# jyakaranda/A-LeGO-LOAM

Hardware: AMD Instinct MI355X
Metric: scans/sec (16x1800 LiDAR) full IP->LO->LM loop (higher is better)
Workload: dtype f32/f64

## Files before the change

a-lego-loam_amd/csrc/alego_api.hip:

```cpp
#include <hip/hip_runtime.h>

#include <cmath>
#include <cstdio>
#include <cstdlib>
#include <algorithm>
#include <cstring>
#include <mutex>
#include <string>
#include <vector>

#include "../../include/alego_mi355x.h"
#include "dev_common.h"
#include "guard_alloc.h"
#include "lm_host.h"
#include "prof.h"
#include "voxel.h"

thread_local Profiler* g_prof = nullptr;


void launch_ip(const DevCtx& d, int ring_pos, bool want_labels, hipStream_t st);
void launch_fe(const DevCtx& d, hipStream_t st);
void launch_lo(const DevCtx& d, hipStream_t st);
void launch_lo_grid(const DevCtx& d, hipStream_t st);
// ... 1166 lines not shown
  hipSetDevice(h->device);
  return lm_host_map_get_keyframe(h->lm, slot, id, out, &h->err);
}
int alego_map_assemble(alego_handle* h, int slot, int kinds, float leaf, alego_point* out, int32_t cap) {
  if (int r = check_slot(h, slot)) return r;
  hipSetDevice(h->device);
  g_prof = &h->prof;
  return lm_host_map_assemble(h->lm, slot, kinds, leaf, out, cap, &h->err);
}
int alego_map_get_stamps(alego_handle* h, int slot, int32_t first, int32_t n, double* out) {
  if (int r = check_slot(h, slot)) return r;
  hipSetDevice(h->device);
  return lm_host_map_stamps(h->lm, slot, first, n, out, 0, &h->err);
}
int alego_map_set_stamps(alego_handle* h, int slot, int32_t first, int32_t n, const double* stamps) {
  if (int r = check_slot(h, slot)) return r;
  hipSetDevice(h->device);
  return lm_host_map_stamps(h->lm, slot, first, n, const_cast<double*>(stamps), 1, &h->err);
}
int alego_map_keyposes(alego_handle* h, int slot, alego_point* out, int32_t cap) {
  if (int r = check_slot(h, slot)) return r;
  hipSetDevice(h->device);
  return lm_host_map_keyposes(h->lm, slot, out, cap, &h->err);
}
int alego_lm_get_local_map(alego_handle* h, int slot, alego_point* corner, int32_t corner_cap, alego_point* surf, int32_t surf_cap, int32_t n_out[2]) {
  if (int r = check_slot(h, slot)) return r;
  if (!n_out || corner_cap < 0 || surf_cap < 0) return ALEGO_ERR_ARG;
  hipSetDevice(h->device);
  return lm_host_get_local_map(h->lm, slot, corner, corner_cap, surf, surf_cap, n_out, &h->err);
}
int alego_voxel_grid(alego_handle* h, const alego_point* pts, int32_t n, float leaf, alego_point* out, int32_t cap) {
  if (!h || n < 0 || cap < 0 || (n > 0 && !pts) || !(leaf > 0.f)) return ALEGO_ERR_ARG;
  hipSetDevice(h->device);
  g_prof = &h->prof;
  return lm_host_voxel_grid(h->lm, h->stream, pts, n, leaf, out, cap, &h->err);
}

int alego_debug_get(alego_handle* h, int slot, const char* name, void* out, int cap_bytes, int* count, int* dtype) {
  if (int r = check_slot(h, slot)) return r;
  hipSetDevice(h->device);
  const DevCtx& d = h->d;
  int sc[SC_COUNT];
  HIP_TRY(h, hipMemcpyAsync(sc, d.scal + (size_t)slot * SC_COUNT, sizeof(sc), hipMemcpyDeviceToHost, stream_of(h, slot)));
  HIP_TRY(h, hipStreamSynchronize(stream_of(h, slot)));
  const std::string s(name);
  const size_t base = (size_t)slot * d.N;
  const int M = sc[SC_M];
  const int cur = sc[SC_CUR];
  int fc[8];
  HIP_TRY(h, hipMemcpy(fc, d.feat_cnt + (size_t)slot * 8, sizeof(fc), hipMemcpyDeviceToHost));
  const void* src = nullptr;
  size_t n = 0;
  int dt = 0, esz = 4;
  auto set = [&](const void* p, size_t cnt, int t) { src = p; n = cnt; dt = t; esz = t == 1 ? 8 : t == 3 ? 1 : 4; };
  if (s == "range_img") set(d.range_img + base, d.N, 0);
  else if (s == "label_img") set(d.label_img + base, d.N, 2);
  else if (s == "flag_img") set(d.flag_img + base, d.N, 3);
  else if (s == "owner") set(d.owner + base, d.N, 2);
  else if (s == "parent") set(d.parent + base, d.N, 2);
  else if (s == "seg_cloud") set(d.seg_pts + base, (size_t)M * 4, 0);
  else if (s == "outlier") set(d.outlier + base, (size_t)sc[SC_NOUT] * 4, 0);
  else if (s == "undistorted" && d.P.deskew_mode) set(d.seg_dsk + base, (size_t)sc[SC_M_DSK] * 4, 0);
  else if (s == "imu_ptr") set(d.imu_ptr + (size_t)slot * 4, 3, 2);
  else if (s == "imu_ring") set(d.imu_ring + (size_t)slot * ALEGO_IMU_Q * 10, ALEGO_IMU_Q * 10, 1);
  else if (s == "seg_ground") set(d.seg_ground + base, M, 3);
  else if (s == "seg_col") set(d.seg_col + base, M, 2);
  else if (s == "seg_range") set(d.seg_range + base, M, 0);
  else if (s == "ring_start") set(d.ring_start + (size_t)slot * d.NS, d.NS, 2);
  else if (s == "ring_end") set(d.ring_end + (size_t)slot * d.NS, d.NS, 2);
  else if (s == "orientation") set(d.ori + (size_t)slot * 4, 3, 0);
  else if (s == "scal") set(d.scal + (size_t)slot * SC_COUNT, SC_COUNT, 2);
  else if (s == "curv_d") set(d.cd + base, M, 0);
  else if (s == "picked_occl") set(d.picked0 + base, M, 3);
  else if (s == "point_label") set(d.plabel + base, M, 2);
  else if (s == "sharp") set(d.feat[0] + ((size_t)slot * 2 + cur) * d.fcap[0], (size_t)fc[cur * 4 + 0] * 4, 0);
  else if (s == "less_sharp") set(d.feat[1] + ((size_t)slot * 2 + cur) * d.fcap[1], (size_t)fc[cur * 4 + 1] * 4, 0);
  else if (s == "flat") set(d.feat[2] + ((size_t)slot * 2 + cur) * d.fcap[2], (size_t)fc[cur * 4 + 2] * 4, 0);
  else if (s == "less_flat") set(d.feat[3] + ((size_t)slot * 2 + cur) * d.fcap[3], (size_t)fc[cur * 4 + 3] * 4, 0);
  else if (s == "sharp_idx") set(d.feat_idx[0] + ((size_t)slot * 2 + cur) * d.fcap[0], fc[cur * 4 + 0], 2);
  else if (s == "less_sharp_idx") set(d.feat_idx[1] + ((size_t)slot * 2 + cur) * d.fcap[1], fc[cur * 4 + 1], 2);
  else if (s == "flat_idx") set(d.feat_idx[2] + ((size_t)slot * 2 + cur) * d.fcap[2], fc[cur * 4 + 2], 2);
  else if (s == "lo_surf_corr") set(d.lo_corr + (size_t)slot * (d.lo_qcap_surf + d.lo_qcap_corner) * 4, (size_t)fc[cur * 4 + 2] * 4, 2);
  else if (s == "lo_corner_corr") set(d.lo_corr + ((size_t)slot * (d.lo_qcap_surf + d.lo_qcap_corner) + d.lo_qcap_surf) * 4, (size_t)fc[cur * 4 + 0] * 4, 2);
  else if (s == "lo_state") set(d.lo_state + (size_t)slot * LO_STATE_N, LO_STATE_N, 1);
  else if (s == "poses") set(d.poses + (size_t)slot * 16, 16, 1);
  else return lm_host_debug_get(h->lm, slot, name, out, cap_bytes, count, dtype, &h->err);
  if ((size_t)cap_bytes < n * esz) { h->err = "debug_get: buffer too small"; return ALEGO_ERR_CAPACITY; }
  if (n) HIP_TRY(h, hipMemcpy(out, src, n * esz, hipMemcpyDeviceToHost));
  *count = (int)n; *dtype = dt;
  return 0;
}

}
```

a-lego-loam_amd/csrc/kernels_fe2.hip:

```cpp
#include <algorithm>
#include <cstdlib>
#include "dev_common.h"
#include "prof.h"
#include "vgrid.h"

#define FE_MAXH 4096

#ifndef FF_G
#define FF_G 4
#endif
#define FF_LPR (64 / FF_G)
#define FF_HALO 8
#define FF_Q0 64
#ifndef FC_NW
#define FC_NW 4
#endif

struct FfLayout {
  int scap, mch, wave_bytes;
};
__host__ __device__ inline FfLayout ff_layout(int sector_cap) {
  FfLayout L;
  L.scap = (FF_Q0 + sector_cap + FF_HALO + 63) & ~63;
  L.mch = L.scap / 64 + 1;
// ... 213 lines not shown
    uint32_t bk = 0u, bp = 0u;
    for (int t = gl; t < nwave; t += FF_LPR) {
      if (act && t < ncand) {
        const uint2 e = lp[t * dir];
        const bool take = FLAT ? e.x > bk : e.x >= bk;
        bk = take ? e.x : bk; bp = take ? e.y : bp;
      }
    }
    const uint32_t kmax = group_max_u32<64 / FF_G>(bk);
    act = act && kmax != 0u;
    if (!__any(act)) break;
    uint32_t pm = group_max_u32<64 / FF_G>(bk == kmax ? bp : 0u);
    if (FLAT) pm = ~pm;
    const int c = (int)(pm >> 6), rf = (int)((pm >> 3) & 7u), rb = (int)(pm & 7u);
    picked += act ? 1 : 0;
    int lab;
    bool spread, more;
    ff_label<FLAT>(P, picked, nmax, lab, spread, more);
    const int lo = max(c - (spread ? rb : 0), 0), hi = c + (spread ? rf : 0);
    const bool rem = act && (FLAT || lab != 0);
    for (int t = gl; t < nwave; t += FF_LPR) {
      if (rem && t < ncand) {
        const uint32_t pv = lp[t * dir].y, loc = (FLAT ? ~pv : pv) >> 6;
        if (loc - (uint32_t)lo <= (uint32_t)(hi - lo)) lp[t * dir].x = 0u;
      }
    }
    ff_commit<FLAT>(R, rem, lab, c, lo, hi, mark, mw, gl);
    act = act && more;
  }
}

#define FF_MW_MAX 28
template <bool BIG>
__global__ void __launch_bounds__(64) fe_pickc(DevCtx d, int sector_cap) {
  const int slot = blockIdx.y + d.slot0, ring0 = blockIdx.x * FF_G, lane = threadIdx.x;
  const int g = lane / FF_LPR, gl = lane % FF_LPR;
  const int NS = d.NS;
  const alego_params& P = d.P;
  int* sc = d.scal + slot * SC_COUNT;
  __shared__ uint32_t s_mark[FF_G][FF_MW_MAX];
  const int mw = min((sector_cap + FF_HALO + 31) / 32 + 1, FF_MW_MAX);
  if (blockIdx.x == 0 && lane == 0) { sc[SC_FE_EPOCH] = sc[SC_FE_EPOCH] + 1; sc[SC_FE_TICKET] = 0; }
  const int ring = ring0 + g;
  const bool rv = ring < NS;
  const int rc = rv ? ring : 0;
  const int S = rv ? d.ring_start[slot * NS + ring] : 0, E = rv ? d.ring_end[slot * NS + ring] : 0;
  int* st = d.st_idx + ((size_t)slot * NS + rc) * d.st_stride;
  const int* cc = ff_counts(d, slot, rc);
  FfPick R;
  R.act0 = false; R.sp = 0; R.carry = -1; R.carry_in = -1; R.n_sharp = 0; R.n_ls = 0; R.n_flat = 0;
  R.st_sharp = st; R.st_lsharp = st + d.cap_sharp; R.st_flat = st + d.cap_sharp + d.cap_lsharp;
  uint32_t* mk = s_mark[g];
  const int NSEC = P.n_sectors;
  for (int j = 0; j < NSEC; ++j) {
    int sp = 0, ep = -1;
    if (rv) ff_sector(P, S, E, j, sp, ep);
    R.act0 = rv && sp < ep; R.sp = sp; R.carry_in = R.carry;
    const int ns = R.act0 ? cc[2 * j] : 0, nf = R.act0 ? cc[2 * j + 1] : 0;
    uint2* lst = ff_list(d, slot, rc, j, sector_cap);
    for (int w = gl; w < mw; w += FF_LPR) mk[w] = 0u;
    const int nsw = (int)wave_max_u32((uint32_t)ns), nfw = (int)wave_max_u32((uint32_t)nf);
    constexpr int KU = 32 / FF_LPR;
    if (nsw <= (BIG ? 64 : 32)) ff_pick_regs<(BIG ? 2 : 1) * KU, false>(P, R, ns, lst, 1, mk, mw, gl);
    else if (nsw <= (BIG ? 128 : 64)) ff_pick_regs<(BIG ? 4 : 2) * KU, false>(P, R, ns, lst, 1, mk, mw, gl);
    else if (nsw <= (BIG ? 192 : 96) && !d.opt_fe_cand) ff_pick_regs<(BIG ? 6 : 3) * KU, false>(P, R, ns, lst, 1, mk, mw, gl);
    else ff_pick_mem<false>(P, R, ns, nsw, lst, 1, mk, mw, gl);
    __builtin_amdgcn_wave_barrier();
    if (nfw <= 32 && !(d.opt_fe_cand && nfw > 8)) ff_pick_regs<KU, true>(P, R, nf, lst + sector_cap - 1, -1, mk, mw, gl);
    else if (BIG && nfw <= 64 && !d.opt_fe_cand) ff_pick_regs<2 * KU, true>(P, R, nf, lst + sector_cap - 1, -1, mk, mw, gl);
    else ff_pick_mem<true>(P, R, nf, nfw, lst + sector_cap - 1, -1, mk, mw, gl);
    __builtin_amdgcn_wave_barrier();
  }
  if (rv && gl == 0) {
    int* c = d.st_cnt + ((size_t)slot * NS + ring) * 8;
    c[0] = R.n_sharp; c[1] = R.n_ls; c[2] = R.n_flat;
  }
}

#ifndef FO_BLOCK
#define FO_BLOCK 256
#endif
#define FO_NB 256
#define FO_U 4
#define FO_CAP_PCT 72
#define FO_INVALID 0xFFFFFFFFu
#define FO_END 0xFFFFu
#define FO_SPIN_LIMIT (1 << 22)
#define FO_ALIAS_INTS (6 * ((FE_MAXH + LO_CH - 1) / LO_CH) > 768 ? 6 * ((FE_MAXH + LO_CH - 1) / LO_CH) : 768)
#define FO_STATIC_LDS (928 + 4 * FO_ALIAS_INTS)
#ifndef FO_BUDGET_BIG
#define FO_BUDGET_BIG 53248
#endif
#ifndef FO_KEYED
#define FO_KEYED 1
#endif
#ifndef FO_STAGE
#define FO_STAGE 0
#endif
struct FoLayout { int cap; int keyed; };
__host__ __device__ inline FoLayout fo_layout(int H) {
  const int budget = 12 * H + FO_STATIC_LDS > 40960 ? FO_BUDGET_BIG : 40960;
  FoLayout L;
  L.keyed = FO_KEYED && 14 * H + FO_STATIC_LDS <= budget;
  const int by_pct = (H * FO_CAP_PCT / 100 + 15) & ~15, by_lds = (budget - FO_STATIC_LDS - (L.keyed ? 14 : 12) * H) / 16;
  L.cap = !FO_STAGE || by_lds <= 0 ? 0 : (by_pct < by_lds ? by_pct : (by_lds & ~15));
  return L;
}
static size_t fo_lds_bytes(int H) { const FoLayout L = fo_layout(H); return std::max((size_t)(L.keyed ? 14 : 12) * H + (size_t)16 * L.cap, (size_t)6 * 65 * 4); }

DEV_INLINE uint32_t mad_u24(uint32_t a, uint32_t b, uint32_t c) { uint32_t r; asm("v_mad_u32_u24 %0, %1, %2, %3" : "=v"(r) : "v"(a), "v"(b), "v"(c)); return r; }

DEV_INLINE uint32_t fo_ord(float f) { const uint32_t b = (uint32_t)d_f2i(f); return b ^ ((b >> 31) ? 0xFFFFFFFFu : 0x80000000u); }
DEV_INLINE float fo_unord(uint32_t u) { return d_i2f((int32_t)(u ^ ((u >> 31) ? 0x80000000u : 0xFFFFFFFFu))); }

#ifdef ALEGO_TIMING
__device__ long long fo_times[24];
extern "C" void alego_fo_times(long long* out) { (void)hipMemcpyFromSymbol(out, HIP_SYMBOL(fo_times), sizeof(long long) * 24); }
#ifndef FO_TICK_RING
#define FO_TICK_RING 8
#endif
#define FO_TICK(k) do { if (threadIdx.x == 0 && ring == FO_TICK_RING && blockIdx.x == 0) fo_times[k] = wall_clock64(); } while (0)
#elif defined(FO_STOP_AFTER)
#define FO_TICK(k) do { if ((k) == FO_STOP_AFTER) { if (threadIdx.x == 0) __hip_atomic_store(&d.fe_sync[(size_t)slot * NS + ring], (epoch << 16), __ATOMIC_RELAXED, __HIP_MEMORY_SCOPE_AGENT); return; } } while (0)
#else
#define FO_TICK(k)
#endif

DEV_INLINE void fo_picks_out(const DevCtx& d, int slot, unsigned char* smem) {
  const int tid = threadIdx.x, NS = d.NS;
  const size_t base = (size_t)slot * d.N;
  const size_t fb = (size_t)slot * 2 + cur_in_flight(d, slot);
  const int* allc = d.st_cnt + (size_t)slot * NS * 8;
  const float4* seg = d.seg_lo + base;
  int (*s_off)[65] = reinterpret_cast<int (*)[65]>(smem);
  if (tid < 64) {
    const int r = tid;
    int c[4];
    c[0] = r < NS ? allc[r * 8 + 0] : 0; c[1] = r < NS ? allc[r * 8 + 1] : 0; c[2] = r < NS ? allc[r * 8 + 2] : 0;
    c[3] = (c[1] + LO_CH - 1) / LO_CH;
#pragma unroll
    for (int k = 0; k < 4; ++k) {
      const int incl = wave_incl_scan(c[k]);
      s_off[k][r] = incl - c[k];
      if (r == 63) s_off[k][64] = incl;
    }
  }
  __syncthreads();
  if (tid <= NS) {
    d.ring_off[(fb * 2) * (NS + 1) + tid] = tid < NS ? s_off[1][tid] : s_off[1][64];
    d.ring_boff[(fb * 2) * (NS + 1) + tid] = tid < NS ? s_off[3][tid] : s_off[3][64];
  }
  if (tid < 3) d.feat_cnt[fb * 4 + tid] = s_off[tid][64];
  auto ring_of = [&](int k, int i) -> int {
    int lo = 0, hi = NS - 1;
    while (lo < hi) { const int mid = (lo + hi + 1) >> 1; if (s_off[k][mid] <= i) lo = mid; else hi = mid - 1; }
    return lo;
  };
  const int stoff[3] = {0, d.cap_sharp, d.cap_sharp + d.cap_lsharp};
#pragma unroll
  for (int k = 0; k < 3; ++k) {
    float4* dst = d.feat[k] + fb * d.fcap[k];
    int* dsti = d.feat_idx[k] + fb * d.fcap[k];
    float4* bx = d.lo_box + (fb * 2 + 1) * d.lo_box_cap * 2;
    const bool boxes = k == F_LSHARP;
    const int nwork = boxes ? s_off[3][64] * LO_CH : s_off[k][64];
    for (int i0 = 0; i0 < nwork; i0 += FO_BLOCK) {
      int i = i0 + tid, r = 0, j = 0, bxi = 0;
      bool v = i < nwork;
      if (boxes) {
        bxi = min(i / LO_CH, s_off[3][64] - 1);
        r = ring_of(3, bxi); j = (bxi - s_off[3][r]) * LO_CH + (tid % LO_CH);
        v = v && j < s_off[k][r + 1] - s_off[k][r];
        i = s_off[k][r] + j;
      } else if (v) { r = ring_of(k, i); j = i - s_off[k][r]; }
      float4 p = make_float4(0.f, 0.f, 0.f, 0.f);
      if (v) {
        const int idx = d.st_idx[((size_t)slot * NS + r) * d.st_stride + stoff[k] + j];
        p = seg[idx];
        dsti[i] = idx; dst[i] = p;
      }
      if (boxes) {
        float mn[3] = {3.402823466e+38f, 3.402823466e+38f, 3.402823466e+38f}, mx[3] = {-3.402823466e+38f, -3.402823466e+38f, -3.402823466e+38f};
        if (v) { mn[0] = mx[0] = p.x; mn[1] = mx[1] = p.y; mn[2] = mx[2] = p.z; }
#pragma unroll
        for (int a = 0; a < 3; ++a)
          bfly_minmax_f32<LO_CH>(mn[a], mx[a]);
        if ((tid % LO_CH) == 0 && v) {
          bx[2 * bxi] = make_float4(mn[0], mn[1], mn[2], __int_as_float(i));
          bx[2 * bxi + 1] = make_float4(mx[0], mx[1], mx[2], __int_as_float(min(LO_CH, s_off[k][r + 1] - i)));
        }
      }
    }
  }
  if (d.n_launch == 1) {
    const int M = d.scal[slot * SC_COUNT + SC_M];
    for (int k = tid; k < M; k += FO_BLOCK) d.plabel[base + k] = 0;
    __syncthreads();
    for (int pass = 0; pass < 3; ++pass) {
      const int k = pass == 0 ? 1 : (pass == 1 ? 0 : 2), lab = pass == 0 ? 1 : (pass == 1 ? 2 : -1);
      for (int i = tid; i < s_off[k][64]; i += FO_BLOCK) {
        const int r = ring_of(k, i);
        d.plabel[base + d.st_idx[((size_t)slot * NS + r) * d.st_stride + stoff[k] + i - s_off[k][r]]] = lab;
      }
      __syncthreads();
    }
  }
}

__global__ void __launch_bounds__(FO_BLOCK) fe_ring_out(DevCtx d) {
  const int slot = blockIdx.x + d.slot0, tid = threadIdx.x, lane = tid & 63;
  const int NS = d.NS, H = d.H;
  extern __shared__ __attribute__((aligned(16))) unsigned char fo_smem[];
  if ((int)blockIdx.x >= d.n_launch) return;
  if ((int)blockIdx.y == NS) { fo_picks_out(d, slot, fo_smem); return; }
  int* scv = d.scal + slot * SC_COUNT;
  __shared__ int s_ticket;
  if (tid == 0) s_ticket = atomicAdd(&scv[SC_FE_TICKET], 1);
  __syncthreads();
  const int ring = min(s_ticket, NS - 1);
  const size_t base = (size_t)slot * d.N;
  const alego_params& P = d.P;
  const int cur = cur_in_flight(d, slot);
  const size_t fb = (size_t)slot * 2 + cur;
  const unsigned epoch = (unsigned)scv[SC_FE_EPOCH] & 0xFFFFu;
  const int S = d.ring_start[slot * NS + ring], E = d.ring_end[slot * NS + ring];
  const int n_all = min(max(E - S, 0), H);
  const int n_ls = d.st_cnt[((size_t)slot * NS + ring) * 8 + 1];
  const int* st_ls = d.st_idx + ((size_t)slot * NS + ring) * d.st_stride + d.cap_sharp;
  const float4* seg = d.seg_lo + base;
  float4* s_pt = reinterpret_cast<float4*>(fo_smem);
  const FoLayout lay = fo_layout(H);
  const int cap = lay.cap;
  unsigned char* fv2 = fo_smem + (size_t)16 * cap;
  uint32_t* s_key = reinterpret_cast<uint32_t*>(fv2);
  uint16_t* s_tmp = reinterpret_cast<uint16_t*>(fv2);
  uint32_t* k_tmp = reinterpret_cast<uint32_t*>(fv2);
  uint16_t* s_order = reinterpret_cast<uint16_t*>(fv2 + (lay.keyed ? 12 : 2) * (size_t)H);
  uint32_t* s_rvid = reinterpret_cast<uint32_t*>(fv2 + 4 * (size_t)H);
  uint16_t* s_rstart = reinterpret_cast<uint16_t*>(fv2 + 8 * (size_t)H);
  uint16_t* s_nxt = reinterpret_cast<uint16_t*>(fv2 + 10 * (size_t)H);
  __shared__ uint32_t s_bm[FE_MAXH / 32 + 2];
  constexpr int FO_MAXBOX = (FE_MAXH + LO_CH - 1) / LO_CH;
  constexpr int FO_ALIAS = FO_ALIAS_INTS;
  static_assert(6 * FO_MAXBOX <= FO_ALIAS && 2 * (FO_NB + 1) <= FO_ALIAS && FE_MAXH / 32 + 1 <= FO_ALIAS, "s_alias holds the bucket tables, the hole prefix or the box corners");
  __shared__ int s_alias[FO_ALIAS];
  int* s_boff = s_alias; int* s_bcur = s_alias + FO_NB + 1; int* s_wpre = s_alias;
  uint32_t* s_bx = reinterpret_cast<uint32_t*>(s_alias);
  __shared__ float s_red[6][FO_BLOCK / 64];
  __shared__ int s_scan[FO_BLOCK / 64], s_cntv[FO_BLOCK / 64];
  __shared__ int s_look[3];
  __shared__ int s_rc[64];
  static_assert(FE_MAXH / 64 <= 64 && FO_BLOCK % 64 == 0, "s_rc holds one count per 64 positions of a ring");
  constexpr int NW = FO_BLOCK / 64;
  const int wv = tid >> 6;
  const unsigned long long lt = (1ull << lane) - 1ull;
  if (tid < 64) s_rc[tid] = 0;
  FO_TICK(0);
  float4 keep[FO_U];
#pragma unroll
  for (int u = 0; u < FO_U; ++u) keep[u] = (seg + S)[(unsigned)max(min(tid + u * FO_BLOCK, n_all - 1), 0)];
  const int BW = (n_all + 31) / 32;
  for (int w = tid; w <= BW + 1 && w <= FE_MAXH / 32 + 1; w += FO_BLOCK) s_bm[w] = 0u;
  __syncthreads();
  for (int t = tid; t < n_ls; t += FO_BLOCK) {
    const int i = st_ls[t] - S;
    if (i >= 0 && i < n_all) atomicOr(&s_bm[i >> 5], 1u << (i & 31));
  }
  if (tid < P.n_sectors) {
    int sp, ep;
    ff_sector(P, S, E, tid, sp, ep);
    const int i = sp - S;
    if (sp == ep && i >= 0 && i < n_all) atomicOr(&s_bm[i >> 5], 1u << (i & 31));
  }
  __syncthreads();
  FO_TICK(1);
  auto hole = [&](int i) -> bool { return (s_bm[i >> 5] >> (i & 31)) & 1u; };
  auto prev_kept = [&](int i) -> int {
    uint32_t w = ~s_bm[i >> 5] & (0xFFFFFFFFu >> (31 - (i & 31)));
    int k = i >> 5;
    while (w == 0u && k > 0) { --k; w = ~s_bm[k]; }
    return w ? k * 32 + 31 - __clz((int)w) : -1;
  };
  auto next_kept = [&](int i) -> int {
    const int j = i + 1;
    uint32_t w = ~s_bm[j >> 5] & (0xFFFFFFFFu << (j & 31));
    int k = j >> 5;
    while (w == 0u && k <= BW) { ++k; w = ~s_bm[k]; }
    return w ? k * 32 + __ffs((int)w) - 1 : n_all;
  };
  const float4* seg_ring = seg + S;
#if FO_STAGE
  auto point = [&](int i) -> float4 { if (i < cap) return s_pt[i]; return seg_ring[(unsigned)i]; };
#else
  auto point = [&](int i) -> float4 { return seg_ring[(unsigned)i]; };
#endif
  const float inv = 1.0f / P.less_flat_leaf;
  float mn[3] = {3.402823466e+38f, 3.402823466e+38f, 3.402823466e+38f}, mx[3] = {-3.402823466e+38f, -3.402823466e+38f, -3.402823466e+38f};
  auto wg_box = [&](int nv) -> int {
    nv = wave_sum_i32(nv);
#pragma unroll
    for (int a = 0; a < 3; ++a) { mn[a] = wave_min_f32(mn[a]); mx[a] = wave_max_f32(mx[a]); }
    __syncthreads();
    if (lane == 0) {
      s_cntv[wv] = nv;
#pragma unroll
      for (int a = 0; a < 3; ++a) { s_red[a][wv] = mn[a]; s_red[3 + a][wv] = mx[a]; }
    }
    __syncthreads();
    nv = 0;
#pragma unroll
    for (int w = 0; w < NW; ++w) nv += s_cntv[w];
#pragma unroll
    for (int a = 0; a < 3; ++a) {
      mn[a] = s_red[a][0]; mx[a] = s_red[3 + a][0];
#pragma unroll
      for (int w = 1; w < NW; ++w) { mn[a] = fminf(mn[a], s_red[a][w]); mx[a] = fmaxf(mx[a], s_red[3 + a][w]); }
    }
    return nv;
  };
  auto bbox_exact = [&]() {
#pragma unroll
    for (int a = 0; a < 3; ++a) { mn[a] = 3.402823466e+38f; mx[a] = -3.402823466e+38f; }
#pragma nounroll
    for (int i = tid; i < n_all; i += FO_BLOCK) {
      if (hole(i)) continue;
      vgr_box_add(mn, mx, point(i));
    }
    (void)wg_box(0);
  };
  int nval = 0;
  {
    int nh = 0;
    for (int w = tid; w <= BW; w += FO_BLOCK) nh += __popc(s_bm[w]);
    for (int i0 = tid; i0 < n_all; i0 += FO_BLOCK * FO_U) {
      float4 pt[FO_U];
#pragma unroll
      for (int u = 0; u < FO_U; ++u) pt[u] = i0 == tid ? keep[u] : seg_ring[(unsigned)min(i0 + u * FO_BLOCK, n_all - 1)];
#pragma unroll
      for (int u = 0; u < FO_U; ++u) {
#if FO_STAGE
        const int i = i0 + u * FO_BLOCK;
        if (i < min(n_all, cap)) s_pt[i] = pt[u];
#endif
        vgr_box_add(mn, mx, pt[u]);
      }
    }
    nval = n_all - wg_box(nh);
  }
  FO_TICK(2);
  bool passthrough = false;
  if (nval > 0 && vgr_leaf_too_small(mn, mx, inv)) { bbox_exact(); passthrough = vgr_leaf_too_small(mn, mx, inv); }
  int nout = 0, nrv = 0, nruns = 0, vex = 0;
  if (passthrough) {
    if (tid == 0) { int acc = 0; for (int w = 0; w <= BW; ++w) { s_wpre[w] = acc; acc += __popc(s_bm[w]); } }
    nout = nval;
  } else if (nval > 0) {
    const VgrGeom g = vgr_geom(mn, mx, inv);
    const bool u24 = (unsigned)g.divb[0] < (1u << 24) && (unsigned)g.divb[1] < (1u << 24) && (unsigned)g.divb[2] < (1u << 24) && g.mul2 < (1u << 24);
    auto key_chunk = [&](int c, float4 own) {
      const int i = c * FO_BLOCK + tid;
      uint32_t key = FO_INVALID;
      if (i < n_all) {
        const int src = prev_kept(i);
        float4 q = own;
        if (src != i) q = point(max(src, 0));
        int i0, i1, i2;
        vgr_coords(g, q, inv, &i0, &i1, &i2);
        const uint32_t id = u24 ? mad_u24((uint32_t)i2, g.mul2, mad_u24((uint32_t)i1, g.mul1, (uint32_t)i0)) : (uint32_t)i0 + (uint32_t)i1 * g.mul1 + (uint32_t)i2 * g.mul2;
        key = src < 0 ? FO_INVALID : id;
        s_key[i] = key;
      }
      const uint32_t prev = (uint32_t)__builtin_amdgcn_update_dpp((int)key, (int)key, 0x138, 0xF, 0xF, false);
      const unsigned long long m = __ballot(i < n_all && key != prev);
      if (lane == 0) s_rc[c * NW + wv] = (int)__popcll(m);
    };
#pragma unroll
    for (int c = 0; c < FO_U; ++c) if (c * FO_BLOCK < n_all) key_chunk(c, keep[c]);
#pragma nounroll
    for (int c = FO_U; c * FO_BLOCK < n_all; ++c) key_chunk(c, seg_ring[(unsigned)min(c * FO_BLOCK + tid, n_all - 1)]);
    __syncthreads();
    {
      const int p0 = lane * 64;
      const int ex = wave_excl_scan(s_rc[lane] + ((p0 < n_all && (p0 == 0 || s_key[p0] != s_key[p0 - 1])) ? 1 : 0), &nruns);
#pragma nounroll
      for (int c = 0; c * FO_BLOCK < n_all; ++c) {
        const int i = c * FO_BLOCK + tid;
        const uint32_t mykey = i < n_all ? s_key[i] : 0u;
        const bool head = i < n_all && (i == 0 || mykey != s_key[i - 1]);
        const unsigned long long m = __ballot(head);
        const int r0 = __builtin_amdgcn_readlane(ex, __builtin_amdgcn_readfirstlane(c * NW + wv));
        if (head) {
          const int r = r0 + (int)__popcll(m & lt);
          s_rvid[r] = mykey;
          s_rstart[r] = (uint16_t)i;
        }
        if (i < n_all) {
          const int j = next_kept(i);
          s_nxt[i] = (uint16_t)((j < n_all && s_key[min(j, n_all - 1)] == mykey) ? j : FO_END);
        }
      }
    }
    __syncthreads();
    FO_TICK(3);
    {
      const unsigned long long T = max(g.T, 1ull);
      int shift = 0;
      while (((T - 1) >> shift) >= (unsigned)FO_NB) ++shift;
      const int nb = (int)((T - 1) >> shift) + 1;
      for (int b = tid; b <= nb; b += FO_BLOCK) s_boff[b] = 0;
      __syncthreads();
      FO_TICK(9);
      for (int r = tid; r < nruns; r += FO_BLOCK) { const uint32_t v = s_rvid[r]; if (v != FO_INVALID) atomicAdd(&s_boff[min((int)(v >> shift), nb - 1) + 1], 1); }
      __syncthreads();
      FO_TICK(10);
      {
        constexpr int PER = FO_NB / FO_BLOCK;
        int v[PER], sum = 0;
#pragma unroll
        for (int k = 0; k < PER; ++k) { const int b = tid * PER + k; v[k] = b < nb ? s_boff[b + 1] : 0; sum += v[k]; }
        const int incl = wave_incl_scan(sum);
        if (lane == 63) s_scan[tid >> 6] = incl;
        __syncthreads();
        int run = incl - sum;
#pragma unroll
        for (int w = 0; w < FO_BLOCK / 64; ++w) if (w < (tid >> 6)) run += s_scan[w];
#pragma unroll
        for (int k = 0; k < PER; ++k) { const int b = tid * PER + k; run += v[k]; if (b < nb) { s_boff[b + 1] = run; s_bcur[b + 1] = run; } }
        if (tid == 0) s_bcur[0] = 0;
      }
      __syncthreads();
      nrv = s_boff[nb];
      FO_TICK(11);
      const bool keyed = lay.keyed && shift <= 20;
      const uint32_t lowmask = (1u << shift) - 1u;
      for (int r = tid; r < nruns; r += FO_BLOCK) {
        const uint32_t v = s_rvid[r];
        if (v != FO_INVALID) {
          const int pos = atomicAdd(&s_bcur[min((int)(v >> shift), nb - 1)], 1);
          if (keyed) k_tmp[pos] = ((v & lowmask) << 12) | (uint32_t)r;
          else s_tmp[pos] = (uint16_t)r;
        }
      }
      __syncthreads();
      FO_TICK(12);
#ifdef ALEGO_TIMING
      if (tid == 0 && ring == FO_TICK_RING && blockIdx.x == 0) { int mxb = 0; for (int b = 0; b < nb; ++b) mxb = max(mxb, s_boff[b + 1] - s_boff[b]); fo_times[16] = n_all; fo_times[17] = nruns; fo_times[18] = nrv; fo_times[19] = nb; fo_times[20] = mxb; }
#endif
      for (int t = tid; t < nrv; t += FO_BLOCK) {
        const uint32_t mine = keyed ? k_tmp[t] : 0u;
        const int r = keyed ? (int)(mine & 0xFFFu) : (int)s_tmp[t];
        const uint32_t v = s_rvid[r];
        const int b = min((int)(v >> shift), nb - 1);
        const int bs = s_boff[b], be = s_boff[b + 1];
        int rank = bs;
        if (keyed) {
#pragma nounroll
          for (int q = bs; q < be; ++q) rank += k_tmp[q] < mine ? 1 : 0;
        } else {
#pragma nounroll
          for (int q = bs; q < be; ++q) { const int o = s_tmp[q]; const uint32_t u = s_rvid[o]; rank += (u < v) || (u == v && o < r); }
        }
        s_order[rank] = (uint16_t)r;
      }
    }
    if (tid < 64) s_rc[tid] = 0;
    __syncthreads();
    FO_TICK(4);
#pragma nounroll
    for (int c = 0; c * FO_BLOCK < nrv; ++c) {
      const int j = c * FO_BLOCK + tid;
      uint32_t st = 0x1000u;
      if (j < nrv) {
        const int r = s_order[j];
        const int i0 = s_rstart[r];
        st = (uint32_t)i0;
        if (j > 0) {
          const int rp = s_order[j - 1];
          if (s_rvid[rp] == s_rvid[r]) {
            int t = (rp + 1 < nruns ? (int)s_rstart[rp + 1] : n_all) - 1;
            while (hole(t)) --t;
            s_nxt[t] = (uint16_t)i0;
// ... 132 lines not shown
```

a-lego-loam_amd/csrc/vgrid.h:

```cpp
#ifndef ALEGO_VGRID_H_
#define ALEGO_VGRID_H_
#include <hip/hip_runtime.h>

__device__ __forceinline__ unsigned vgr_enc(float f) {
  const unsigned b = (unsigned)__float_as_int(f);
  return b ^ ((b >> 31) ? 0xFFFFFFFFu : 0x80000000u);
}
__device__ __forceinline__ float vgr_dec(unsigned u) { return __int_as_float((int)((u >> 31) ? (u ^ 0x80000000u) : ~u)); }
__device__ __forceinline__ void vgr_box_load(const unsigned* bb, float mn[3], float mx[3]) {
#pragma unroll
  for (int a = 0; a < 3; ++a) { mn[a] = vgr_dec(bb[a]); mx[a] = vgr_dec(~bb[4 + a]); }
}

__device__ __forceinline__ void vgr_box_add(float mn[3], float mx[3], float4 p) {
  mn[0] = fminf(mn[0], p.x); mn[1] = fminf(mn[1], p.y); mn[2] = fminf(mn[2], p.z);
  mx[0] = fmaxf(mx[0], p.x); mx[1] = fmaxf(mx[1], p.y); mx[2] = fmaxf(mx[2], p.z);
}

__device__ __forceinline__ bool vgr_leaf_too_small(const float mn[3], const float mx[3], float inv) {
  const long long dx = (long long)((mx[0] - mn[0]) * inv) + 1, dy = (long long)((mx[1] - mn[1]) * inv) + 1, dz = (long long)((mx[2] - mn[2]) * inv) + 1;
  return dx * dy * dz > 2147483647LL;
}

struct VgrGeom {
  int minb[3], divb[3];
  unsigned mul1, mul2;
  unsigned long long T;
};
__device__ __forceinline__ VgrGeom vgr_geom(const float mn[3], const float mx[3], float inv) {
  VgrGeom g;
#pragma unroll
  for (int a = 0; a < 3; ++a) { g.minb[a] = (int)floorf(mn[a] * inv); g.divb[a] = (int)floorf(mx[a] * inv) - g.minb[a] + 1; }
  g.mul1 = (unsigned)g.divb[0];
  g.mul2 = (unsigned)g.divb[0] * (unsigned)g.divb[1];
  g.T = (unsigned long long)(unsigned)g.divb[0] * (unsigned)g.divb[1] * (unsigned)g.divb[2];
  return g;
}
__device__ __forceinline__ int vgr_bits(unsigned long long T) {
  if (T > 0xFFFFFFFFull || T == 0) return 32;
  return T > 1 ? 32 - __clz((int)(unsigned)(T - 1)) : 0;
}
__device__ __forceinline__ void vgr_coords(const VgrGeom& g, float4 p, float inv, int* i0, int* i1, int* i2) {
  *i0 = (int)(floorf(p.x * inv) - (float)g.minb[0]);
  *i1 = (int)(floorf(p.y * inv) - (float)g.minb[1]);
  *i2 = (int)(floorf(p.z * inv) - (float)g.minb[2]);
}
__device__ __forceinline__ unsigned vgr_id(const VgrGeom& g, float4 p, float inv) {
  int i0, i1, i2;
  vgr_coords(g, p, inv, &i0, &i1, &i2);
  return (unsigned)i0 + (unsigned)i1 * g.mul1 + (unsigned)i2 * g.mul2;
}

__device__ __forceinline__ unsigned long long vkey_pack(int ix, int iy, int iz) {
  const int B = 1 << 20;
  const unsigned long long x = (unsigned long long)(unsigned)min(max(ix + B, 0), 2 * B - 1), y = (unsigned long long)(unsigned)min(max(iy + B, 0), 2 * B - 1),
                           z = (unsigned long long)(unsigned)min(max(iz + B, 0), 2 * B - 1);
  return (z << 42) | (y << 21) | x;
}
__device__ __forceinline__ unsigned long long vkey_of(const float4& p, float inv) {
  return vkey_pack((int)floorf(p.x * inv), (int)floorf(p.y * inv), (int)floorf(p.z * inv));
}

#endif
```

a-lego-loam_amd/csrc/wave.h:

```cpp
#ifndef ALEGO_WAVE_H_
#define ALEGO_WAVE_H_
#include <hip/hip_runtime.h>
#include <stdint.h>

__device__ __forceinline__ int lane_id() { return threadIdx.x & 63; }

__device__ __forceinline__ int wave_incl_scan(int x) {
  const int lane = lane_id();
#pragma unroll
  for (int o = 1; o < 64; o <<= 1) { const int t = __shfl_up(x, o, 64); if (lane >= o) x += t; }
  return x;
}
__device__ __forceinline__ int wave_excl_scan(int x, int* total) {
  const int incl = wave_incl_scan(x);
  *total = __builtin_amdgcn_readlane(incl, 63);
  return incl - x;
}
template <int NW>
__device__ __forceinline__ int block_excl_scan(int v, int* s_w, int* total) {
  const int wave = threadIdx.x >> 6;
  const int incl = wave_incl_scan(v);
  __syncthreads();
  if (lane_id() == 63) s_w[wave] = incl;
  __syncthreads();
  int woff = 0, tot = 0;
#pragma unroll
  for (int w = 0; w < NW; ++w) { const int c = s_w[w]; if (w < wave) woff += c; tot += c; }
  *total = tot;
  return woff + incl - v;
}

template <int W = 64>
__device__ __forceinline__ int bfly_sum_i32(int v) {
#pragma unroll
  for (int o = W / 2; o > 0; o >>= 1) v += __shfl_xor(v, o, 64);
  return v;
}
template <int W = 64>
__device__ __forceinline__ int bfly_min_i32(int v) {
#pragma unroll
  for (int o = W / 2; o > 0; o >>= 1) v = min(v, __shfl_xor(v, o, 64));
  return v;
}
template <int W = 64>
__device__ __forceinline__ int bfly_max_i32(int v) {
#pragma unroll
  for (int o = W / 2; o > 0; o >>= 1) v = max(v, __shfl_xor(v, o, 64));
  return v;
}
template <int W = 64>
__device__ __forceinline__ unsigned long long bfly_min_u64(unsigned long long v) {
#pragma unroll
  for (int o = W / 2; o > 0; o >>= 1) v = min(v, (unsigned long long)__shfl_xor(v, o, 64));
  return v;
}
template <int W = 64>
__device__ __forceinline__ void bfly_minmax_f32(float& mn, float& mx) {
#pragma unroll
  for (int o = W / 2; o > 0; o >>= 1) { mn = fminf(mn, __shfl_xor(mn, o, 64)); mx = fmaxf(mx, __shfl_xor(mx, o, 64)); }
}
__device__ __forceinline__ double bfly_sum_f64(double v) {
#pragma unroll
  for (int o = 32; o > 0; o >>= 1) v += __shfl_xor(v, o, 64);
  return v;
}

template <int CTRL>
__device__ __forceinline__ int dpp_max_u32_step(int x) {
  const int t = __builtin_amdgcn_update_dpp(x, x, CTRL, 0xF, 0xF, false);
  return (uint32_t)t > (uint32_t)x ? t : x;
}
template <int G>
__device__ __forceinline__ uint32_t group_max_u32(uint32_t v) {
  static_assert(G == 1 || G == 2 || G == 4 || G == 8 || G == 16, "a DPP group is 1, 2, 4, 8 or 16 lanes");
  int x = (int)v;
  if constexpr (G >= 2) x = dpp_max_u32_step<0xB1>(x);
  if constexpr (G >= 4) x = dpp_max_u32_step<0x4E>(x);
  if constexpr (G >= 8) x = dpp_max_u32_step<0x141>(x);
  if constexpr (G >= 16) x = dpp_max_u32_step<0x140>(x);
  return (uint32_t)x;
}
template <int G>
__device__ __forceinline__ uint32_t group_min_u32(uint32_t v) { return ~group_max_u32<G>(~v); }
template <int G>
__device__ __forceinline__ unsigned long long group_min_u64(unsigned long long v) {
  const uint32_t hi = group_min_u32<G>((uint32_t)(v >> 32));
  const uint32_t lo = group_min_u32<G>((uint32_t)(v >> 32) == hi ? (uint32_t)v : 0xFFFFFFFFu);
  return ((unsigned long long)hi << 32) | lo;
}

__device__ __forceinline__ uint32_t wave_max_u32(uint32_t v) {
  const int x = (int)group_max_u32<16>(v);
  const uint32_t a = (uint32_t)__builtin_amdgcn_readlane(x, 0), b = (uint32_t)__builtin_amdgcn_readlane(x, 16);
  const uint32_t c = (uint32_t)__builtin_amdgcn_readlane(x, 32), e = (uint32_t)__builtin_amdgcn_readlane(x, 48);
  const uint32_t ab = a > b ? a : b, ce = c > e ? c : e;
  return ab > ce ? ab : ce;
}
__device__ __forceinline__ uint32_t wave_min_u32(uint32_t v) { return ~wave_max_u32(~v); }
__device__ __forceinline__ unsigned long long wave_max_u64(unsigned long long v) {
  const uint32_t hi = wave_max_u32((uint32_t)(v >> 32));
  const uint32_t lo = wave_max_u32((uint32_t)(v >> 32) == hi ? (uint32_t)v : 0u);
  return ((unsigned long long)hi << 32) | lo;
}
__device__ __forceinline__ unsigned long long wave_min_u64(unsigned long long v) {
  const uint32_t hi = wave_min_u32((uint32_t)(v >> 32));
  const uint32_t lo = wave_min_u32((uint32_t)(v >> 32) == hi ? (uint32_t)v : 0xFFFFFFFFu);
  return ((unsigned long long)hi << 32) | lo;
}
#define ALEGO_DPP_F32(x, ctrl, rmask) __int_as_float(__builtin_amdgcn_update_dpp(__float_as_int(x), __float_as_int(x), ctrl, rmask, 0xF, false))
__device__ __forceinline__ float wave_min_f32(float x) {
  x = fminf(x, ALEGO_DPP_F32(x, 0xB1, 0xF)); x = fminf(x, ALEGO_DPP_F32(x, 0x4E, 0xF)); x = fminf(x, ALEGO_DPP_F32(x, 0x141, 0xF)); x = fminf(x, ALEGO_DPP_F32(x, 0x140, 0xF));
  x = fminf(x, ALEGO_DPP_F32(x, 0x142, 0xA)); x = fminf(x, ALEGO_DPP_F32(x, 0x143, 0xC));
// ... 17 lines not shown
```

Before: 444,400.

## Restructure less-flat voxel downsample run-building to per-thread contiguous spans

Each thread in the less-flat voxel-filter kernel now owns K contiguous points held in registers. Keys, run heads and next-links are computed locally, with a wave scan and a small cross-wave carry table replacing the s_key staging array, the prev_kept/next_kept bitmap walks and the separate head-scan pass. The bounding-box reduction now uses 16-lane DPP plus LDS atomic min/max/add instead of a two-barrier shared-memory fold. A cheap float test skips the exact bbox path when the grid surely fits, and the inclusive wave scan moves to DPP row shifts. The carry logic is more complex and register pressure rises with K=8. The new debug getters are incidental.

```diff
diff --git a/a-lego-loam_amd/csrc/alego_api.hip b/a-lego-loam_amd/csrc/alego_api.hip
--- a/a-lego-loam_amd/csrc/alego_api.hip
+++ b/a-lego-loam_amd/csrc/alego_api.hip
@@ -1272,6 +1272,10 @@
   else if (s == "flat_idx") set(d.feat_idx[2] + ((size_t)slot * 2 + cur) * d.fcap[2], fc[cur * 4 + 2], 2);
   else if (s == "lo_surf_corr") set(d.lo_corr + (size_t)slot * (d.lo_qcap_surf + d.lo_qcap_corner) * 4, (size_t)fc[cur * 4 + 2] * 4, 2);
   else if (s == "lo_corner_corr") set(d.lo_corr + ((size_t)slot * (d.lo_qcap_surf + d.lo_qcap_corner) + d.lo_qcap_surf) * 4, (size_t)fc[cur * 4 + 0] * 4, 2);
+  else if (s == "st_cnt") set(d.st_cnt + (size_t)slot * d.NS * 8, (size_t)d.NS * 8, 2);
+  else if (s == "less_flat_ring_off") set(d.ring_off + (((size_t)slot * 2 + cur) * 2 + 1) * (d.NS + 1), d.NS + 1, 2);
+  else if (s == "less_flat_ring_boff") set(d.ring_boff + (((size_t)slot * 2 + cur) * 2 + 1) * (d.NS + 1), d.NS + 1, 2);
+  else if (s == "less_flat_box") set(d.lo_box + (((size_t)slot * 2 + cur) * 2 + 0) * d.lo_box_cap * 2, (size_t)((fc[cur * 4 + 3] + LO_CH - 1) / LO_CH + d.NS) * 8, 0);
   else if (s == "lo_state") set(d.lo_state + (size_t)slot * LO_STATE_N, LO_STATE_N, 1);
   else if (s == "poses") set(d.poses + (size_t)slot * 16, 16, 1);
   else return lm_host_debug_get(h->lm, slot, name, out, cap_bytes, count, dtype, &h->err);
diff --git a/a-lego-loam_amd/csrc/kernels_fe2.hip b/a-lego-loam_amd/csrc/kernels_fe2.hip
--- a/a-lego-loam_amd/csrc/kernels_fe2.hip
+++ b/a-lego-loam_amd/csrc/kernels_fe2.hip
@@ -319,7 +319,7 @@
 #endif
 #define FO_NB 256
 #define FO_U 4
-#define FO_CAP_PCT 72
+#define FO_K 8
 #define FO_INVALID 0xFFFFFFFFu
 #define FO_END 0xFFFFu
 #define FO_SPIN_LIMIT (1 << 22)
@@ -331,21 +331,24 @@
 #ifndef FO_KEYED
 #define FO_KEYED 1
 #endif
-#ifndef FO_STAGE
-#define FO_STAGE 0
-#endif
-struct FoLayout { int cap; int keyed; };
+struct FoLayout { int keyed; };
 __host__ __device__ inline FoLayout fo_layout(int H) {
   const int budget = 12 * H + FO_STATIC_LDS > 40960 ? FO_BUDGET_BIG : 40960;
   FoLayout L;
   L.keyed = FO_KEYED && 14 * H + FO_STATIC_LDS <= budget;
-  const int by_pct = (H * FO_CAP_PCT / 100 + 15) & ~15, by_lds = (budget - FO_STATIC_LDS - (L.keyed ? 14 : 12) * H) / 16;
-  L.cap = !FO_STAGE || by_lds <= 0 ? 0 : (by_pct < by_lds ? by_pct : (by_lds & ~15));
   return L;
 }
-static size_t fo_lds_bytes(int H) { const FoLayout L = fo_layout(H); return std::max((size_t)(L.keyed ? 14 : 12) * H + (size_t)16 * L.cap, (size_t)6 * 65 * 4); }
+static size_t fo_lds_bytes(int H) { const FoLayout L = fo_layout(H); return std::max((size_t)(L.keyed ? 14 : 12) * H, (size_t)6 * 65 * 4); }
 
 DEV_INLINE uint32_t mad_u24(uint32_t a, uint32_t b, uint32_t c) { uint32_t r; asm("v_mad_u32_u24 %0, %1, %2, %3" : "=v"(r) : "v"(a), "v"(b), "v"(c)); return r; }
+
+DEV_INLINE void fo_box_merge(uint32_t* red, uint32_t a0, uint32_t a1, uint32_t a2, uint32_t b0, uint32_t b1, uint32_t b2, uint32_t n) {
+  const uint32_t addr = (uint32_t)(uintptr_t)(__attribute__((address_space(3))) uint32_t*)red;
+  asm volatile("ds_min_u32 %0, %1\n\tds_min_u32 %0, %2 offset:4\n\tds_min_u32 %0, %3 offset:8\n\t"
+               "ds_max_u32 %0, %4 offset:12\n\tds_max_u32 %0, %5 offset:16\n\tds_max_u32 %0, %6 offset:20\n\t"
+               "ds_add_u32 %0, %7 offset:24\n\ts_waitcnt lgkmcnt(0)"
+               :: "v"(addr), "v"(a0), "v"(a1), "v"(a2), "v"(b0), "v"(b1), "v"(b2), "v"(n) : "memory");
+}
 
 DEV_INLINE uint32_t fo_ord(float f) { const uint32_t b = (uint32_t)d_f2i(f); return b ^ ((b >> 31) ? 0xFFFFFFFFu : 0x80000000u); }
 DEV_INLINE float fo_unord(uint32_t u) { return d_i2f((int32_t)(u ^ ((u >> 31) ? 0x80000000u : 0xFFFFFFFFu))); }
@@ -465,11 +468,8 @@
   const int n_ls = d.st_cnt[((size_t)slot * NS + ring) * 8 + 1];
   const int* st_ls = d.st_idx + ((size_t)slot * NS + ring) * d.st_stride + d.cap_sharp;
   const float4* seg = d.seg_lo + base;
-  float4* s_pt = reinterpret_cast<float4*>(fo_smem);
   const FoLayout lay = fo_layout(H);
-  const int cap = lay.cap;
-  unsigned char* fv2 = fo_smem + (size_t)16 * cap;
-  uint32_t* s_key = reinterpret_cast<uint32_t*>(fv2);
+  unsigned char* fv2 = fo_smem;
   uint16_t* s_tmp = reinterpret_cast<uint16_t*>(fv2);
   uint32_t* k_tmp = reinterpret_cast<uint32_t*>(fv2);
   uint16_t* s_order = reinterpret_cast<uint16_t*>(fv2 + (lay.keyed ? 12 : 2) * (size_t)H);
@@ -483,21 +483,29 @@
   __shared__ int s_alias[FO_ALIAS];
   int* s_boff = s_alias; int* s_bcur = s_alias + FO_NB + 1; int* s_wpre = s_alias;
   uint32_t* s_bx = reinterpret_cast<uint32_t*>(s_alias);
-  __shared__ float s_red[6][FO_BLOCK / 64];
-  __shared__ int s_scan[FO_BLOCK / 64], s_cntv[FO_BLOCK / 64];
+  __shared__ uint32_t s_red[8];
+  __shared__ int s_scan[FO_BLOCK / 64];
   __shared__ int s_look[3];
+  __shared__ uint16_t s_spare;
   __shared__ int s_rc[64];
   static_assert(FE_MAXH / 64 <= 64 && FO_BLOCK % 64 == 0, "s_rc holds one count per 64 positions of a ring");
   constexpr int NW = FO_BLOCK / 64;
+  constexpr int FO_CW = NW * ((FE_MAXH + FO_BLOCK * FO_K - 1) / (FO_BLOCK * FO_K));
+  static_assert(4 * FO_CW <= 64 && (4 * FO_CW & (4 * FO_CW - 1)) == 0 && FO_K <= 8, "s_cw fits in s_rc; a span's holes are read as one byte of the bitmap");
+  uint32_t* s_cw = reinterpret_cast<uint32_t*>(s_rc);
   const int wv = tid >> 6;
   const unsigned long long lt = (1ull << lane) - 1ull;
-  if (tid < 64) s_rc[tid] = 0;
   FO_TICK(0);
-  float4 keep[FO_U];
-#pragma unroll
-  for (int u = 0; u < FO_U; ++u) keep[u] = (seg + S)[(unsigned)max(min(tid + u * FO_BLOCK, n_all - 1), 0)];
+  const int nsw = max((n_all + FO_BLOCK * FO_K - 1) / (FO_BLOCK * FO_K), 1);
+  const int K = max((n_all + FO_BLOCK * nsw - 1) / (FO_BLOCK * nsw), 1);
+  const float4* seg_ring = seg + S;
+  const int i_last = max(n_all - 1, 0);
+  float4 pt[FO_K];
+#pragma unroll
+  for (int k = 0; k < FO_K; ++k) if (k < K) pt[k] = seg_ring[(unsigned)min(tid * K + k, i_last)];
   const int BW = (n_all + 31) / 32;
   for (int w = tid; w <= BW + 1 && w <= FE_MAXH / 32 + 1; w += FO_BLOCK) s_bm[w] = 0u;
+  if (tid < 8) s_red[tid] = tid < 3 ? 0xFFFFFFFFu : 0u;
   __syncthreads();
   for (int t = tid; t < n_ls; t += FO_BLOCK) {
     const int i = st_ls[t] - S;
@@ -512,50 +520,24 @@
   __syncthreads();
   FO_TICK(1);
   auto hole = [&](int i) -> bool { return (s_bm[i >> 5] >> (i & 31)) & 1u; };
-  auto prev_kept = [&](int i) -> int {
-    uint32_t w = ~s_bm[i >> 5] & (0xFFFFFFFFu >> (31 - (i & 31)));
-    int k = i >> 5;
-    while (w == 0u && k > 0) { --k; w = ~s_bm[k]; }
-    return w ? k * 32 + 31 - __clz((int)w) : -1;
-  };
-  auto next_kept = [&](int i) -> int {
-    const int j = i + 1;
-    uint32_t w = ~s_bm[j >> 5] & (0xFFFFFFFFu << (j & 31));
-    int k = j >> 5;
-    while (w == 0u && k <= BW) { ++k; w = ~s_bm[k]; }
-    return w ? k * 32 + __ffs((int)w) - 1 : n_all;
-  };
-  const float4* seg_ring = seg + S;
-#if FO_STAGE
-  auto point = [&](int i) -> float4 { if (i < cap) return s_pt[i]; return seg_ring[(unsigned)i]; };
-#else
   auto point = [&](int i) -> float4 { return seg_ring[(unsigned)i]; };
-#endif
   const float inv = 1.0f / P.less_flat_leaf;
   float mn[3] = {3.402823466e+38f, 3.402823466e+38f, 3.402823466e+38f}, mx[3] = {-3.402823466e+38f, -3.402823466e+38f, -3.402823466e+38f};
   auto wg_box = [&](int nv) -> int {
-    nv = wave_sum_i32(nv);
-#pragma unroll
-    for (int a = 0; a < 3; ++a) { mn[a] = wave_min_f32(mn[a]); mx[a] = wave_max_f32(mx[a]); }
+    if (__ballot(nv != 0)) nv = wave_sum_i32(nv);
+    uint32_t lo[3], hi[3];
+#pragma unroll
+    for (int a = 0; a < 3; ++a) { lo[a] = group_min_u32<16>(vgr_enc(mn[a])); hi[a] = group_max_u32<16>(vgr_enc(mx[a])); }
+    if ((lane & 15) == 0) fo_box_merge(s_red, lo[0], lo[1], lo[2], hi[0], hi[1], hi[2], lane == 0 ? (uint32_t)nv : 0u);
     __syncthreads();
-    if (lane == 0) {
-      s_cntv[wv] = nv;
-#pragma unroll
-      for (int a = 0; a < 3; ++a) { s_red[a][wv] = mn[a]; s_red[3 + a][wv] = mx[a]; }
-    }
-    __syncthreads();
-    nv = 0;
-#pragma unroll
-    for (int w = 0; w < NW; ++w) nv += s_cntv[w];
-#pragma unroll
-    for (int a = 0; a < 3; ++a) {
-      mn[a] = s_red[a][0]; mx[a] = s_red[3 + a][0];
-#pragma unroll
-      for (int w = 1; w < NW; ++w) { mn[a] = fminf(mn[a], s_red[a][w]); mx[a] = fmaxf(mx[a], s_red[3 + a][w]); }
-    }
-    return nv;
+#pragma unroll
+    for (int a = 0; a < 3; ++a) { mn[a] = vgr_dec(s_red[a]); mx[a] = vgr_dec(s_red[3 + a]); }
+    return (int)s_red[6];
   };
   auto bbox_exact = [&]() {
+    __syncthreads();
+    if (tid < 8) s_red[tid] = tid < 3 ? 0xFFFFFFFFu : 0u;
+    __syncthreads();
 #pragma unroll
     for (int a = 0; a < 3; ++a) { mn[a] = 3.402823466e+38f; mx[a] = -3.402823466e+38f; }
 #pragma nounroll
@@ -569,24 +551,20 @@
   {
     int nh = 0;
     for (int w = tid; w <= BW; w += FO_BLOCK) nh += __popc(s_bm[w]);
-    for (int i0 = tid; i0 < n_all; i0 += FO_BLOCK * FO_U) {
-      float4 pt[FO_U];
-#pragma unroll
-      for (int u = 0; u < FO_U; ++u) pt[u] = i0 == tid ? keep[u] : seg_ring[(unsigned)min(i0 + u * FO_BLOCK, n_all - 1)];
-#pragma unroll
-      for (int u = 0; u < FO_U; ++u) {
-#if FO_STAGE
-        const int i = i0 + u * FO_BLOCK;
-        if (i < min(n_all, cap)) s_pt[i] = pt[u];
-#endif
-        vgr_box_add(mn, mx, pt[u]);
-      }
+#pragma unroll
+    for (int k = 0; k < FO_K; ++k) if (k < K) vgr_box_add(mn, mx, pt[k]);
+    for (int i0 = FO_BLOCK * K + tid; i0 < n_all; i0 += FO_BLOCK * FO_U) {
+      float4 q[FO_U];
+#pragma unroll
+      for (int u = 0; u < FO_U; ++u) q[u] = seg_ring[(unsigned)min(i0 + u * FO_BLOCK, n_all - 1)];
+#pragma unroll
+      for (int u = 0; u < FO_U; ++u) vgr_box_add(mn, mx, q[u]);
     }
     nval = n_all - wg_box(nh);
   }
   FO_TICK(2);
   bool passthrough = false;
-  if (nval > 0 && vgr_leaf_too_small(mn, mx, inv)) { bbox_exact(); passthrough = vgr_leaf_too_small(mn, mx, inv); }
+  if (nval > 0 && !vgr_leaf_surely_fits(mn, mx, inv) && vgr_leaf_too_small(mn, mx, inv)) { bbox_exact(); passthrough = vgr_leaf_too_small(mn, mx, inv); }
   int nout = 0, nrv = 0, nruns = 0, vex = 0;
   if (passthrough) {
     if (tid == 0) { int acc = 0; for (int w = 0; w <= BW; ++w) { s_wpre[w] = acc; acc += __popc(s_bm[w]); } }
@@ -594,46 +572,82 @@
   } else if (nval > 0) {
     const VgrGeom g = vgr_geom(mn, mx, inv);
     const bool u24 = (unsigned)g.divb[0] < (1u << 24) && (unsigned)g.divb[1] < (1u << 24) && (unsigned)g.divb[2] < (1u << 24) && g.mul2 < (1u << 24);
-    auto key_chunk = [&](int c, float4 own) {
-      const int i = c * FO_BLOCK + tid;
-      uint32_t key = FO_INVALID;
-      if (i < n_all) {
-        const int src = prev_kept(i);
-        float4 q = own;
-        if (src != i) q = point(max(src, 0));
+    for (int s = 0; s < nsw; ++s) {
+      const int vw = s * NW + wv;
+      const int b = (s * FO_BLOCK + tid) * K;
+      if (s > 0) {
+#pragma unroll
+        for (int k = 0; k < FO_K; ++k) if (k < K) pt[k] = seg_ring[(unsigned)min(b + k, i_last)];
+      }
+      const uint32_t bw0 = s_bm[b >> 5], bw1 = s_bm[(b >> 5) + 1];
+      const uint32_t holes = (uint32_t)((((unsigned long long)bw1 << 32) | bw0) >> (b & 31));
+      const uint32_t kept = ~holes & ((1u << min(max(n_all - b, 0), K)) - 1u);
+      const bool has = kept != 0u;
+      uint32_t id[FO_K];
+#pragma unroll
+      for (int k = 0; k < FO_K; ++k) if (k < K) {
         int i0, i1, i2;
-        vgr_coords(g, q, inv, &i0, &i1, &i2);
-        const uint32_t id = u24 ? mad_u24((uint32_t)i2, g.mul2, mad_u24((uint32_t)i1, g.mul1, (uint32_t)i0)) : (uint32_t)i0 + (uint32_t)i1 * g.mul1 + (uint32_t)i2 * g.mul2;
-        key = src < 0 ? FO_INVALID : id;
-        s_key[i] = key;
-      }
-      const uint32_t prev = (uint32_t)__builtin_amdgcn_update_dpp((int)key, (int)key, 0x138, 0xF, 0xF, false);
-      const unsigned long long m = __ballot(i < n_all && key != prev);
-      if (lane == 0) s_rc[c * NW + wv] = (int)__popcll(m);
-    };
-#pragma unroll
-    for (int c = 0; c < FO_U; ++c) if (c * FO_BLOCK < n_all) key_chunk(c, keep[c]);
-#pragma nounroll
-    for (int c = FO_U; c * FO_BLOCK < n_all; ++c) key_chunk(c, seg_ring[(unsigned)min(c * FO_BLOCK + tid, n_all - 1)]);
-    __syncthreads();
-    {
-      const int p0 = lane * 64;
-      const int ex = wave_excl_scan(s_rc[lane] + ((p0 < n_all && (p0 == 0 || s_key[p0] != s_key[p0 - 1])) ? 1 : 0), &nruns);
-#pragma nounroll
-      for (int c = 0; c * FO_BLOCK < n_all; ++c) {
-        const int i = c * FO_BLOCK + tid;
-        const uint32_t mykey = i < n_all ? s_key[i] : 0u;
-        const bool head = i < n_all && (i == 0 || mykey != s_key[i - 1]);
-        const unsigned long long m = __ballot(head);
-        const int r0 = __builtin_amdgcn_readlane(ex, __builtin_amdgcn_readfirstlane(c * NW + wv));
-        if (head) {
-          const int r = r0 + (int)__popcll(m & lt);
-          s_rvid[r] = mykey;
-          s_rstart[r] = (uint16_t)i;
+        vgr_coords(g, pt[k], inv, &i0, &i1, &i2);
+        id[k] = u24 ? mad_u24((uint32_t)i2, g.mul2, mad_u24((uint32_t)i1, g.mul1, (uint32_t)i0)) : (uint32_t)i0 + (uint32_t)i1 * g.mul1 + (uint32_t)i2 * g.mul2;
+      }
+      const int kfirst = __ffs((int)kept) - 1;
+      uint32_t fkey = 0u, lkey = 0u;
+      int cnt = 0;
+#pragma unroll
+      for (int k = 0; k < FO_K; ++k) if (k < K) {
+        const bool kp = (kept >> k) & 1u;
+        cnt += (kp && k != kfirst && id[k] != lkey) ? 1 : 0;
+        fkey = k == kfirst ? id[k] : fkey;
+        lkey = kp ? id[k] : lkey;
+      }
+      const int lpos = has ? b + 31 - __clz((int)kept) : -1;
+      const unsigned long long ne = __ballot(has);
+      const int src = wave_prev_lane(ne);
+      int cpos = __shfl(lpos, max(src, 0), 64);
+      uint32_t ckey = (uint32_t)__shfl((int)lkey, max(src, 0), 64);
+      cnt += (has && src >= 0 && fkey != ckey) ? 1 : 0;
+      cnt += (s == 0 && tid == 0 && (holes & 1u)) ? 1 : 0;
+      int wtot;
+      const int ex = wave_excl_scan(cnt, &wtot);
+      const int lf = ne ? __builtin_amdgcn_readfirstlane(__ffsll((unsigned long long)ne) - 1) : 0;
+      const int ll = ne ? __builtin_amdgcn_readfirstlane(63 - __clzll((long long)ne)) : 0;
+      const uint32_t wfkey = (uint32_t)__builtin_amdgcn_readlane((int)fkey, lf), wlkey = (uint32_t)__builtin_amdgcn_readlane((int)lkey, ll);
+      const int wlpos = __builtin_amdgcn_readlane(lpos, ll);
+      if (lane == 0) { s_cw[vw] = (uint32_t)wtot; s_cw[FO_CW + vw] = wfkey; s_cw[2 * FO_CW + vw] = (uint32_t)wlpos; s_cw[3 * FO_CW + vw] = wlkey; }
+      if (has) s_nxt[lpos] = (uint16_t)FO_END;
+      __syncthreads();
+      const int cwv = (int)s_cw[lane & (4 * FO_CW - 1)];
+      const int vwu = __builtin_amdgcn_readfirstlane(vw);
+      int rbase = 0, tot = 0, xpos = -1, open = 0;
+      uint32_t xkey = FO_INVALID;
+      {
+        int rp = -1;
+        uint32_t rk = FO_INVALID;
+#pragma unroll
+        for (int w = 0; w < FO_CW; ++w) if (w < (s + 1) * NW) {
+          const int lp = __builtin_amdgcn_readlane(cwv, 2 * FO_CW + w);
+          const int xh = (lp >= 0 && (rp < 0 || (uint32_t)__builtin_amdgcn_readlane(cwv, FO_CW + w) != rk)) ? 1 : 0;
+          if (w == vwu) { rbase = tot; open = xh; xpos = rp; xkey = rk; }
+          tot += __builtin_amdgcn_readlane(cwv, w) + xh;
+          if (lp >= 0) { rp = lp; rk = (uint32_t)__builtin_amdgcn_readlane(cwv, 3 * FO_CW + w); }
         }
-        if (i < n_all) {
-          const int j = next_kept(i);
-          s_nxt[i] = (uint16_t)((j < n_all && s_key[min(j, n_all - 1)] == mykey) ? j : FO_END);
+      }
+      nruns = tot;
+      if (src < 0) { cpos = xpos; ckey = xkey; }
+      int r = rbase + ex + ((lane > lf) ? open : 0);
+      if (s == 0 && tid == 0 && (holes & 1u)) { s_rvid[0] = FO_INVALID; s_rstart[0] = 0; r = 1; }
+      uint16_t* nx = cpos >= 0 ? s_nxt + cpos : &s_spare;
+      if (cpos < 0) ckey = ~fkey;
+      uint32_t* rv = s_rvid + r;
+      uint16_t* rs = s_rstart + r;
+#pragma unroll
+      for (int k = 0; k < FO_K; ++k) if (k < K) {
+        if ((kept >> k) & 1u) {
+          const int pos = b + k;
+          const bool head = id[k] != ckey;
+          *nx = (uint16_t)(head ? FO_END : pos);
+          if (head) { *rv++ = id[k]; *rs++ = (uint16_t)pos; }
+          nx = s_nxt + pos; ckey = id[k];
         }
       }
     }
diff --git a/a-lego-loam_amd/csrc/vgrid.h b/a-lego-loam_amd/csrc/vgrid.h
--- a/a-lego-loam_amd/csrc/vgrid.h
+++ b/a-lego-loam_amd/csrc/vgrid.h
@@ -20,6 +20,10 @@
 __device__ __forceinline__ bool vgr_leaf_too_small(const float mn[3], const float mx[3], float inv) {
   const long long dx = (long long)((mx[0] - mn[0]) * inv) + 1, dy = (long long)((mx[1] - mn[1]) * inv) + 1, dz = (long long)((mx[2] - mn[2]) * inv) + 1;
   return dx * dy * dz > 2147483647LL;
+}
+__device__ __forceinline__ bool vgr_leaf_surely_fits(const float mn[3], const float mx[3], float inv) {
+  const float ex = (mx[0] - mn[0]) * inv + 1.0f, ey = (mx[1] - mn[1]) * inv + 1.0f, ez = (mx[2] - mn[2]) * inv + 1.0f;
+  return ex >= 1.0f && ey >= 1.0f && ez >= 1.0f && ex * ey * ez < 1073741824.0f;
 }
 
 struct VgrGeom {
diff --git a/a-lego-loam_amd/csrc/wave.h b/a-lego-loam_amd/csrc/wave.h
--- a/a-lego-loam_amd/csrc/wave.h
+++ b/a-lego-loam_amd/csrc/wave.h
@@ -6,9 +6,9 @@
 __device__ __forceinline__ int lane_id() { return threadIdx.x & 63; }
 
 __device__ __forceinline__ int wave_incl_scan(int x) {
-  const int lane = lane_id();
-#pragma unroll
-  for (int o = 1; o < 64; o <<= 1) { const int t = __shfl_up(x, o, 64); if (lane >= o) x += t; }
+  x += __builtin_amdgcn_update_dpp(0, x, 0x111, 0xF, 0xF, false); x += __builtin_amdgcn_update_dpp(0, x, 0x112, 0xF, 0xF, false);
+  x += __builtin_amdgcn_update_dpp(0, x, 0x114, 0xF, 0xF, false); x += __builtin_amdgcn_update_dpp(0, x, 0x118, 0xF, 0xF, false);
+  x += __builtin_amdgcn_update_dpp(0, x, 0x142, 0xA, 0xF, false); x += __builtin_amdgcn_update_dpp(0, x, 0x143, 0xC, 0xF, false);
   return x;
 }
 __device__ __forceinline__ int wave_excl_scan(int x, int* total) {
@@ -28,6 +28,11 @@
   for (int w = 0; w < NW; ++w) { const int c = s_w[w]; if (w < wave) woff += c; tot += c; }
   *total = tot;
   return woff + incl - v;
+}
+
+__device__ __forceinline__ int wave_prev_lane(unsigned long long m) {
+  const unsigned long long below = m & ((1ull << lane_id()) - 1ull);
+  return below ? 63 - __clzll((long long)below) : -1;
 }
 
 template <int W = 64>
```

Result: no change. 448,700 (median of 6 runs) (+1.0%).
